# polixir/emei

Measured on AMD Instinct MI355X. Metric: env-steps/s, higher is better.
Workload: dtype f64

## Files before the change

### emei_amd/csrc/abi.hip

```cpp
#include <hip/hip_runtime.h>

#include <cmath>
#include <cstdarg>
#include <cstdio>
#include <cstring>
#include <ctime>
#include <new>

#include "launch.h"
#include "body_kernels.h"
#include "cheetah_model.h"
#include "hopper_model.h"
#include "dpend_model.h"

using namespace emei;

struct emei_env {
    emei_config cfg;
    int obs_dim, act_dim, state_dim;
    size_t real_size;
    void* state;
    int32_t* steps;
    uint32_t* episode;
    unsigned long long* done_mask;
    void* frozen_state;
    int32_t* frozen_steps;
    uint32_t* frozen_episode;
    uint64_t frozen_seed;
    unsigned long long* cap_hits;
    uint32_t* work;
    int resident_waves;
    bool has_state, frozen;
    int last_kernel;
    uint32_t* host_flag = nullptr;
    uint32_t flag_seq = 0;
    PendParams pend;
    const void* trig;
    ObsPeers peers;
};

static thread_local char g_err[512] = "";

static int fail(int code, const char* fmt, ...) {
    va_list ap;
    va_start(ap, fmt);
    vsnprintf(g_err, sizeof(g_err), fmt, ap);
// ... 60 lines not shown
    if (!out || capacity < 0) return fail(EMEI_ERR_INVALID, "emei_model_invweights: bad argument");
    double buf[32];
    int n;
    switch (env_id) {
        case EMEI_IP_REBOUND_BALANCING:
        case EMEI_IP_BOUNDARY_BALANCING:
        case EMEI_IP_REBOUND_SWINGUP:
        case EMEI_IP_BOUNDARY_SWINGUP: {
            constexpr IpModel m = ip_make_model(false);
            buf[0] = m.invw, buf[1] = m.invw_hinge, n = 2;
            break;
        }
        case EMEI_IDP_REBOUND_BALANCING:
        case EMEI_IDP_BOUNDARY_BALANCING:
        case EMEI_IDP_REBOUND_SWINGUP:
        case EMEI_IDP_BOUNDARY_SWINGUP: buf[0] = dpend::make_model(false, 0.002).invw, n = 1; break;
        case EMEI_HALFCHEETAH_RUNNING: n = cheetah::xml_invweights(buf); break;
        case EMEI_HOPPER_RUNNING: n = hopper::xml_invweights(buf); break;
        case EMEI_CARTPOLE_SWINGUP:
        case EMEI_CARTPOLE_BALANCING: return fail(EMEI_ERR_UNSUPPORTED, "emei_model_invweights: CartPole has no constraint rows");
        default: return fail(EMEI_ERR_INVALID, "unknown env_id %d", env_id);
    }
    if (n > capacity) return fail(EMEI_ERR_INVALID, "emei_model_invweights: %d values, capacity %d", n, capacity);
    memcpy(out, buf, n * sizeof(double));
    return n;
}

#include <cstddef>
#include <mutex>
namespace emei {
const void* emei_trig_table(int device) {
// ... 41 lines not shown
    p.dt = dt;
    p.dt32 = (float)dt;
    for (int i = 0; i < 4; ++i) p.init_sigma[i] = init_sigma ? init_sigma[i] : 0.f;
    p.noise_shared = noise_shared;
    const bool swingup = env_id == EMEI_IP_REBOUND_SWINGUP || env_id == EMEI_IP_BOUNDARY_SWINGUP;
    const IpModel x = ip_make_model(swingup);
    p.M11 = x.M11, p.M22 = x.M22, p.mpr = x.mpr, p.mgr = x.mp * x.gravity * x.r;
    p.gear = x.gear, p.ctrl_lo = x.ctrl_lo, p.ctrl_hi = x.ctrl_hi, p.x_lo = x.x_lo, p.x_hi = x.x_hi;
    p.phi_off = x.phi_off, p.sin_off = x.sin_off, p.cos_off = x.cos_off;
    p.invw = x.invw;
    p.tc = x.solref_tc < 2 * dt ? 2 * dt : x.solref_tc;
    p.dampratio = 1.0, p.dmin = x.dmin, p.dmax = x.dmax, p.width = x.width;
    p.limK = 1.0 / (p.dmax * p.dmax * p.tc * p.tc * p.dampratio * p.dampratio), p.limB = 2.0 / (p.dmax * p.tc);
    return p;
}

extern "C" EMEI_API int emei_create(const emei_config* cfg, emei_env** out) {
    if (!cfg || !out) return fail(EMEI_ERR_INVALID, "emei_create: null argument");
    const uint32_t size_v2a = (uint32_t)offsetof(emei_config, env_param_mask);
    const uint32_t size_v5 = (uint32_t)offsetof(emei_config, ode_method);
    if (cfg->struct_size != sizeof(emei_config) && cfg->struct_size != size_v5 && cfg->struct_size != size_v2a &&
        cfg->struct_size != EMEI_CONFIG_SIZE_V1)
        return fail(EMEI_ERR_INVALID, "emei_create: emei_config size %u, library expects %zu (or the older sizes %u / %u / %u)",
                    cfg->struct_size, sizeof(emei_config), size_v5, size_v2a, EMEI_CONFIG_SIZE_V1);
    emei_config c2;
    memset(&c2, 0, sizeof(c2));
    memcpy(&c2, cfg, cfg->struct_size);
    if (cfg->struct_size == EMEI_CONFIG_SIZE_V1)
        for (int i = 0; i < EMEI_MAX_STATE_DIM; ++i) c2.init_sigma[i] = (float)c2.init_noise;
    c2.struct_size = sizeof(emei_config);
// ... 29 lines not shown
    if (cfg->max_episode_steps < 0) return fail(EMEI_ERR_INVALID, "emei_create: max_episode_steps < 0");
    int prev_device = 0;
    HIP_TRY(hipGetDevice(&prev_device));
    HIP_TRY(hipSetDevice(cfg->device));
    struct RestoreDevice {
        int d;
        ~RestoreDevice() { (void)hipSetDevice(d); }
    } restore{prev_device};

    emei_env* h = new (std::nothrow) emei_env();
    if (!h) return fail(EMEI_ERR_INVALID, "emei_create: out of host memory");
    memset(h, 0, sizeof(*h));
    h->cfg = *cfg;
    h->obs_dim = od, h->act_dim = ad, h->state_dim = sd;
    h->real_size = cfg->precision == EMEI_PRECISION_F32 ? sizeof(float) : sizeof(double);
    const size_t n = (size_t)cfg->n_envs, n_words = (n + kWave - 1) / kWave;
    const size_t state_bytes = n * sd * h->real_size;
    hipError_t e = hipSuccess;
    if (e == hipSuccess) e = hipMalloc(&h->state, state_bytes);
    if (e == hipSuccess) e = hipMalloc((void**)&h->steps, n * sizeof(int32_t));
    if (e == hipSuccess) e = hipMalloc((void**)&h->episode, n * sizeof(uint32_t));
    if (e == hipSuccess) e = hipMalloc((void**)&h->done_mask, n_words * sizeof(unsigned long long));
    if (e == hipSuccess) e = hipMalloc(&h->frozen_state, state_bytes);
    if (e == hipSuccess) e = hipMalloc((void**)&h->frozen_steps, n * sizeof(int32_t));
    if (e == hipSuccess) e = hipMalloc((void**)&h->frozen_episode, n * sizeof(uint32_t));
    if (e == hipSuccess) e = hipMalloc((void**)&h->cap_hits, sizeof(unsigned long long));
    if (e == hipSuccess) e = hipMemset(h->cap_hits, 0, sizeof(unsigned long long));
    if (e == hipSuccess && steps_as_body(*cfg)) {
        e = hipMalloc((void**)&h->work, (2 + 2 * n_words) * sizeof(uint32_t));
        if (e == hipSuccess) e = hipMemset(h->work, 0, (2 + 2 * n_words) * sizeof(uint32_t));
// ... 1 lines not shown
    if (e == hipSuccess) e = hipMemset(h->done_mask, 0, n_words * sizeof(unsigned long long));
    if (e == hipSuccess) e = hipMemset(h->steps, 0, n * sizeof(int32_t));
    if (e == hipSuccess) e = hipMemset(h->episode, 0, n * sizeof(uint32_t));
    if (e != hipSuccess) {
        emei_destroy(h);
        return fail(EMEI_ERR_HIP, "emei_create: allocation failed: %s", hipGetErrorString(e));
    }
    if (is_pend(cfg->env_id))
        h->pend = pend_params(cfg->env_id, cfg->real_time_scale, cfg->init_sigma, cfg->noise_layout);
    h->trig = emei_trig_table(cfg->device);
    if (!h->trig) {
        emei_destroy(h);
        return fail(EMEI_ERR_HIP, "emei_create: could not build the trig table on device %d", cfg->device);
    }
    if (steps_as_body(*cfg)) {
        BodyLaunch L;
        L.op = BODY_OP_OCCUPANCY, L.env_id = cfg->env_id, L.precision = cfg->precision, L.integrator = cfg->integrator;
        L.solver = (int)cfg->solver, L.selected = &h->resident_waves;
        if (body_launch(L) != EMEI_OK) h->resident_waves = 0;
    }
    *out = h;
    return EMEI_OK;
}

extern "C" EMEI_API int emei_destroy(emei_env* h) {
    if (!h) return EMEI_OK;
    (void)hipFree(h->state);
    (void)hipFree(h->steps);
    (void)hipFree(h->episode);
    (void)hipFree(h->done_mask);
    (void)hipFree(h->frozen_state);
    (void)hipFree(h->frozen_steps);
    (void)hipFree(h->frozen_episode);
// ... 49 lines not shown
    L.freq_rate = h->cfg.freq_rate;
    L.max_episode_steps = h->cfg.max_episode_steps;
    L.seed = h->cfg.seed;
    L.env_offset = h->cfg.env_index_offset;
    L.dt = h->cfg.real_time_scale;
    L.integrator = h->cfg.integrator;
    L.solver = (int)h->cfg.solver;
    memcpy(L.noise.init, h->cfg.init_sigma, sizeof(L.noise.init));
    memcpy(L.noise.obs, h->cfg.obs_sigma, sizeof(L.noise.obs));
    L.noise.shared = h->cfg.noise_layout == EMEI_NOISE_SHARED;
    L.env_params.mask = h->cfg.env_param_mask;
    memcpy(L.env_params.v, h->cfg.env_params, sizeof(L.env_params.v));
    L.trig = h->trig;
    L.cap_hits = h->cap_hits;
    L.work = h->work, L.chunk_steps = h->cfg.rollout_chunk_steps, L.resident_waves = h->resident_waves;
    L.stream = (hipStream_t)stream;
    return L;
}

extern "C" EMEI_API int emei_reset(emei_env* h, uint64_t seed, void* stream) {
    if (!h) return fail(EMEI_ERR_INVALID, "emei_reset: null handle");
    EMEI_ON_DEVICE(h, "emei_reset");
    h->cfg.seed = seed;
    int rc;
    if (is_pend(h->cfg.env_id)) {
        PendLaunch L = pend_base(h, stream);
        L.op = PEND_OP_RESET;
        rc = pend_launch(L);
    } else {
        BodyLaunch L = body_base(h, stream);
// ... 764 lines not shown
```

### emei_amd/csrc/body_kernels.h

```cpp
#pragma once
#include "emei_device.h"

namespace emei {

struct EnvParams {
    uint32_t mask = 0;
    double v[EMEI_MAX_ENV_PARAMS] = {0};
    double get(int k, double dflt) const { return (mask >> k) & 1u ? v[k] : dflt; }
};

struct NoiseSpec {
    float init[EMEI_MAX_STATE_DIM] = {0}, obs[EMEI_MAX_STATE_DIM] = {0};
    int32_t shared = 0;
};
template <int NS>
struct NoiseArgs {
    float init[NS], obs[NS];
    int32_t shared, obs_on;
    NoiseArgs() = default;
    explicit NoiseArgs(const NoiseSpec& h) : shared(h.shared), obs_on(0) {
        for (int i = 0; i < NS; ++i) init[i] = h.init[i], obs[i] = h.obs[i], obs_on |= h.obs[i] != 0.f;
    }
};
constexpr uint64_t kObsNoiseKey = 0x6F62736E6F697365ull;
// ... 19 lines not shown
        boxmuller(r.v[2], r.v[3], z[4 * b + 2], z[4 * b + 3]);
    }
#pragma unroll
    for (int i = 0; i < NS; ++i) {
        const R d = (R)__fmul_rn(sig[i], z[i]);
        s[i] = ASSIGN ? d : s[i] + d;
    }
}
template <class Body>
__device__ __forceinline__ void body_init(typename Body::real (&s)[Body::NS], uint64_t seed, uint64_t env, uint32_t episode,
                                          const NoiseArgs<Body::NS>& ns) {
    gauss_state<typename Body::real, Body::NS, true>(s, seed, env, episode, 0u, ns.init, ns.shared != 0);
    Body::init_base(s);
}

template <class Body, bool RK4>
__device__ __forceinline__ void body_substep(typename Body::real (&s)[Body::NS], const typename Body::real (&ctrl)[Body::NA],
                                             const typename Body::Model& m, bool semi, const TrigCtx& trig,
                                             typename Body::Warm& warm) {
    using R = typename Body::real;
    constexpr int NV = Body::NS / 2;
    const R dt = (R)m.dt;
    R q[NV], v[NV], acc[NV];
#pragma unroll
    for (int i = 0; i < NV; ++i) q[i] = s[i], v[i] = s[NV + i];
    if constexpr (!RK4) {
        typename Body::Warm cold{};
        Body::accel(q, v, ctrl, m, dt, acc, trig, cold);
#pragma unroll
        for (int i = 0; i < NV; ++i) {
            const R vn = fma_r(dt, acc[i], v[i]);
            s[i] = fma_r(dt, semi ? vn : v[i], q[i]);
            s[NV + i] = vn;
        }
    } else {
        R qs[NV], vs[NV], dq[NV], dv[NV];
#pragma unroll
        for (int i = 0; i < NV; ++i) qs[i] = q[i], vs[i] = v[i], dq[i] = R(0), dv[i] = R(0);
        Body::begin_stages(warm);
        auto stage = [&](int st) __attribute__((always_inline)) {
            Body::accel(qs, vs, ctrl, m, R(0), acc, trig, warm);
            const R b = (st == 0 || st == 3) ? R(1.0 / 6.0) : R(1.0 / 3.0);
            const R h = dt * (st == 2 ? R(1) : R(0.5));
#pragma unroll
            for (int i = 0; i < NV; ++i) {
                dq[i] = fma_r(b, vs[i], dq[i]), dv[i] = fma_r(b, acc[i], dv[i]);
                qs[i] = fma_r(h, vs[i], q[i]);
// ... 34 lines not shown
    uint8_t* done_out = nullptr;
    int64_t n = 0;
    int32_t n_steps = 1, freq_rate = 1, max_episode_steps = 0;
    uint32_t flags = 0;
    uint64_t seed = 0, env_offset = 0;
    double dt = 0.002;
    int32_t integrator = 0;
    int32_t solver = 0;
    NoiseSpec noise;
    EnvParams env_params;
    const void* trig = nullptr;
    unsigned long long* cap_hits = nullptr;
    uint32_t* work = nullptr;
    int32_t chunk_steps = 0;
    int32_t resident_waves = 0;
    hipStream_t stream = nullptr;
    int* selected = nullptr;
    const double* start_rows = nullptr;
    int32_t n_candidates = 1;
    double discount = 1.0;
    double* return_out = nullptr;
    int32_t* length_out = nullptr;
    CandidateSpec cand = {};
    void* partials = nullptr;
    const float* sigma_map = nullptr;
};
int body_launch(const BodyLaunch& L);

template <class Body>
struct BodyArgs {
// ... 48 lines not shown
    }
};

template <class Body>
__host__ __device__ constexpr int rollout_block() {
#ifdef EMEI_BODY_BLOCK
    return EMEI_BODY_BLOCK;
#else
    return Body::kMinWavesPerEU == 1 ? kWave : kBlock;
#endif
}

#ifndef EMEI_WORKQUEUE
#define EMEI_WORKQUEUE 1
#endif
template <class Body, bool RK4, bool QUEUE = false>
__global__ void __launch_bounds__(rollout_block<Body>()) __attribute__((amdgpu_waves_per_eu(Body::kMinWavesPerEU)))
    body_rollout_kernel(const BodyArgs<Body> a) {
    static_assert(!QUEUE || rollout_block<Body>() == kWave, "work items are one-wave blocks");
    using R = typename Body::real;
    constexpr int NS = Body::NS, NO = Body::NO, NA = Body::NA;
    constexpr int kBlock = rollout_block<Body>();
    constexpr int kWaves = kBlock / kWave;
    constexpr int kActVec = (kWave * NA + 3) / 4, kObsVec = (kWave * NO + 3) / 4;
    constexpr int kActIt = (kActVec + kWave - 1) / kWave, kObsIt = (kObsVec + kWave - 1) / kWave;
    __shared__ __attribute__((aligned(16))) float act_s[kWaves][kActIt * kWave * 4];
    __shared__ __attribute__((aligned(16))) float obs_s[kWaves][kObsIt * kWave * 4];
    __shared__ SinCosEntry trig_s[kTrigTableSize];
    stage_trig_table<kBlock>(trig_s, a.trig);
    TrigCtx trig;
    trig.tab = trig_s;
    __shared__ R scratch_s[(Body::kScratchPerLane > 0 ? Body::kScratchPerLane : 1) * (Body::kScratchPerLane > 0 ? kBlock : 1)];
    if constexpr (Body::kScratchPerLane > 0) trig.scratch = scratch_s;
    trig.scratch_stride = kBlock;
// ... 48 lines not shown
    const int wave_envs = (int)min((int64_t)kWave, n - i0);
    const bool active = i < n;

    R s[NS];
    int32_t steps = 0;
    uint32_t episode = 0;
    if (active) {
#pragma unroll
        for (int k = 0; k < NS; ++k) s[k] = a.state[(int64_t)k * n + i];
        steps = a.steps[i];
        episode = a.episode[i];
    } else {
        Body::park(s);
    }
    const bool auto_reset = (a.flags & EMEI_FLAG_AUTO_RESET) != 0;
    const bool obs_noise = a.noise.obs_on != 0;
    uint32_t done = 0;
    R spare[Body::kSpareReset ? NS : 1];
    bool have_spare = false;

    float4 av[kActIt];
    auto fetch_actions = [&](int t) __attribute__((always_inline)) {
        const float* base = a.actions + ((int64_t)t * n + i0) * NA;
        const bool fast = wave_envs == kWave && (((uintptr_t)base) & 15u) == 0;
#pragma unroll
        for (int c = 0; c < kActIt; ++c) {
            const int vec = c * kWave + lane;
            av[c] = make_float4(0.f, 0.f, 0.f, 0.f);
            if (fast) {
                if (vec < kActVec) av[c] = ((const float4*)base)[vec];
            } else {
// ... 17 lines not shown
        } else {
#pragma unroll
            for (int c = 0; c < kActIt; ++c) ((float4*)act_s[wv])[c * kWave + lane] = av[c];
            wave_lds_fence();
#pragma unroll
            for (int k = 0; k < NA; ++k) ctrl[k] = (R)act_s[wv][lane * NA + k];
            wave_lds_fence();
            if (t + 1 < t_end) fetch_actions(t + 1);
        }

        R pre[NS];
#pragma unroll
        for (int k = 0; k < NS; ++k) pre[k] = s[k];
        typename Body::Warm warm{};
        for (int k = 0; k < a.freq_rate; ++k) {
            body_substep<Body, RK4>(s, ctrl, a.m, a.semi != 0, trig, warm);
            if (obs_noise)
                gauss_state<R, NS, false>(s, a.seed ^ kObsNoiseKey, a.env_offset + (uint64_t)i, episode,
                                          ((uint32_t)steps * (uint32_t)a.freq_rate + (uint32_t)k) * (uint32_t)((NS + 3) / 4),
                                          a.noise.obs, a.noise.shared != 0);
        }
        EMEI_MARK(step_io);
        float o[NO];
        R rew;
        bool term;
        Body::outputs(s, pre, ctrl, a.m, a.freq_rate, o, rew, term, trig);
        ++steps;
        const bool trunc = (a.max_episode_steps > 0) & (steps >= a.max_episode_steps);
        done = active ? ((term ? EMEI_DONE_TERMINAL : 0u) | (trunc ? EMEI_DONE_TRUNCATED : 0u)) : 0u;

        if (a.obs_out) {
            float* mine = &obs_s[wv][lane * NO];
#pragma unroll
            for (int k = 0; k < NO; ++k) mine[k] = o[k];
            wave_lds_fence();
// ... 249 lines not shown
                if constexpr (!DRAWN) {
                    ret_out[j] = ret;
                    len_out[j] = t + 1;
                    if (final_obs) {
#pragma unroll
                        for (int k = 0; k < NO; ++k) final_obs[j * NO + k] = o[k];
                    }
                }
            }
        }
        if (__ballot(live) == 0ull) break;
    }
    if constexpr (DRAWN) plan_reduce_wave(j, nk, i, n_cand, ret, len, partials);
    if constexpr (DRAWN && KEEP) {
        if (active) ret_out[j] = ret;
    }
}

template <class Body>
static int launch_body(const BodyLaunch& L) {
    using R = typename Body::real;
    const typename Body::Model m = Body::make_model(L.dt, L.env_params);
    dim3 grid((unsigned)((L.n + kBlock - 1) / kBlock));
    dim3 rgrid((unsigned)((L.n + rollout_block<Body>() - 1) / rollout_block<Body>()));
    switch (L.op) {
        case BODY_OP_ROLLOUT: {
            BodyArgs<Body> a;
            a.state = (R*)L.state, a.steps = L.steps, a.episode = L.episode, a.done_mask = L.done_mask;
            a.actions = (const float*)L.actions, a.obs_out = L.obs_out, a.reward_out = L.reward_out, a.done_out = L.done_out;
            a.n = L.n, a.n_steps = L.n_steps, a.freq_rate = L.freq_rate, a.max_episode_steps = L.max_episode_steps;
// ... 3 lines not shown
            a.cap_hits = L.cap_hits;
            a.work = nullptr, a.chunk_steps = 0, a.n_waves = rgrid.x, a.n_items = 0;
            if constexpr (rollout_block<Body>() == kWave && EMEI_WORKQUEUE != 0) {
                int cs = L.chunk_steps;
                if (cs == 0) cs = (L.resident_waves > 0 && (int64_t)rgrid.x > L.resident_waves) ? -((kGuidedMin << 4) | kGuidedShift) : 0;
                else if (cs <= -100) cs = -(((-cs / 100) << 4) | max(1, min(-cs % 100, 6)));
                else if (cs < 0) cs = 0;
                const unsigned n_chunks = cs != 0 ? WorkQueue::count_chunks(L.n_steps, cs) : 1u;
                if (L.work && n_chunks > 1 && (uint64_t)rgrid.x * n_chunks < (1ull << 31)) {
                    static_assert(WorkQueue::kProgress == WorkQueue::kTicket + 1, "one memset");
                    if (hipMemsetAsync(L.work + WorkQueue::kTicket, 0, (size_t)(1 + rgrid.x) * sizeof(uint32_t), L.stream) != hipSuccess)
                        return EMEI_ERR_HIP;
                    a.work = L.work, a.chunk_steps = cs, a.n_items = rgrid.x * n_chunks;
                    const unsigned workers = L.resident_waves > 0 ? (unsigned)L.resident_waves : 1024u;
                    rgrid.x = min(workers, a.n_items);
                    if (L.integrator == EMEI_INTEG_RK4)
                        hipLaunchKernelGGL((body_rollout_kernel<Body, true, true>), rgrid, dim3(kWave), 0, L.stream, a);
                    else
                        hipLaunchKernelGGL((body_rollout_kernel<Body, false, true>), rgrid, dim3(kWave), 0, L.stream, a);
                }
            }
            if (!a.work) {
                if (L.integrator == EMEI_INTEG_RK4)
                    hipLaunchKernelGGL((body_rollout_kernel<Body, true>), rgrid, dim3(rollout_block<Body>()), 0, L.stream, a);
                else
                    hipLaunchKernelGGL((body_rollout_kernel<Body, false>), rgrid, dim3(rollout_block<Body>()), 0, L.stream, a);
            }
            if (L.selected)
                *L.selected = a.work ? (L.integrator == EMEI_INTEG_RK4 ? EMEI_KERNEL_BODY_RK4_CHUNKED : EMEI_KERNEL_BODY_CHUNKED)
                                     : (L.integrator == EMEI_INTEG_RK4 ? EMEI_KERNEL_BODY_RK4 : EMEI_KERNEL_BODY);
            break;
        }
        case BODY_OP_OCCUPANCY: {
            int dev = 0, cus = 0, nb = 0;
            if (hipGetDevice(&dev) != hipSuccess || hipDeviceGetAttribute(&cus, hipDeviceAttributeMultiprocessorCount, dev) != hipSuccess)
                return EMEI_ERR_HIP;
            hipError_t e;
            if constexpr (rollout_block<Body>() == kWave && EMEI_WORKQUEUE != 0) {
                e = L.integrator == EMEI_INTEG_RK4
                        ? hipOccupancyMaxActiveBlocksPerMultiprocessor(&nb, body_rollout_kernel<Body, true, true>, rollout_block<Body>(), 0)
                        : hipOccupancyMaxActiveBlocksPerMultiprocessor(&nb, body_rollout_kernel<Body, false, true>, rollout_block<Body>(), 0);
            } else {
                e = L.integrator == EMEI_INTEG_RK4
                        ? hipOccupancyMaxActiveBlocksPerMultiprocessor(&nb, body_rollout_kernel<Body, true>, rollout_block<Body>(), 0)
                        : hipOccupancyMaxActiveBlocksPerMultiprocessor(&nb, body_rollout_kernel<Body, false>, rollout_block<Body>(), 0);
            }
            if (e != hipSuccess) return EMEI_ERR_HIP;
            if (L.selected) *L.selected = nb * cus * (rollout_block<Body>() / kWave);
            return EMEI_OK;
        }
        case BODY_OP_RESET:
            hipLaunchKernelGGL(body_reset_kernel<Body>, grid, dim3(kBlock), 0, L.stream, (R*)L.state, L.steps, L.episode,
                               L.n, L.seed, L.env_offset, NoiseArgs<Body::NS>(L.noise));
            break;
        case BODY_OP_GET_OBS:
            hipLaunchKernelGGL(body_get_obs_kernel<Body>, grid, dim3(kBlock), 0, L.stream, (const R*)L.state, L.obs_f64,
                               L.n, m);
            break;
        case BODY_OP_INIT_OBS:
            hipLaunchKernelGGL(body_init_obs_kernel<Body>, grid, dim3(kBlock), 0, L.stream, L.env_index, L.episode_in,
                               L.obs_out, L.n, L.seed, L.env_offset, NoiseArgs<Body::NS>(L.noise), m);
// ... 110 lines not shown
```

### emei_amd/csrc/cheetah_model.h

```cpp
#pragma once
#include <cmath>
#include <cstring>
#include <type_traits>

#include "constexpr_math.h"
#include "emei_device.h"

namespace emei {
namespace cheetah {

constexpr int NV = 9;
enum { P_BFOOT = 0, P_BSHIN = 1, P_BTHIGH = 2, P_FFOOT = 3, P_FSHIN = 4, P_FTHIGH = 5, P_TORSO = 6, P_X = 7, P_Z = 8 };

__host__ __device__ constexpr bool nz(int i, int j) { return i >= 6 || (i / 3) == (j / 3); }

struct Model {
    double sx[7], sz[7], diag[7];
    double d_tb[2], d_tf[2], d_bt_bs[2], d_bs_bf[2], d_ft_fs[2], d_fs_ff[2];
    double mtot, gravity, z0;
    double stiff[6], damp[6], arm[6], lo[6], hi[6], gear[6];
    double geom_end[16][2];
    double radius, friction;
    double cK, cB, c_dmin, c_dmax, c_width;
    double lK, lB, l_dmin, l_dmax, l_width;
// ... 1124 lines not shown
    qacc[6] = a[P_FTHIGH] - a[P_TORSO], qacc[7] = a[P_FSHIN] - a[P_FTHIGH], qacc[8] = a[P_FFOOT] - a[P_FSHIN];
}

}

template <typename R, int SOLVER = EMEI_SOLVER_NEWTON>
struct CheetahBody {
    using real = R;
    using Model = cheetah::Model;
    static constexpr int kMinWavesPerEU = 1;
#ifndef EMEI_CHEETAH_UNROLL_RK4
#define EMEI_CHEETAH_UNROLL_RK4 1
#endif
    static constexpr bool kUnrollRK4 = EMEI_CHEETAH_UNROLL_RK4 != 0;
    static constexpr int kScratchPerLane = SOLVER == EMEI_SOLVER_NEWTON ? cheetah::kDualSlots * cheetah::kSlotFields : 0;
    static constexpr bool kHasCtrlCost = true;
    static constexpr bool kObsIsState = true;
    static constexpr bool kSpareReset = false;
    static constexpr bool kStreamOutputs = false;
    static constexpr int NS = 18, NO = 18, NA = 6;
    static Model make_model(double dt, const EnvParams& ep) {
        Model m = cheetah::cheetah_make_model(dt);
        m.w_forward = ep.get(EMEI_PARAM_FORWARD_REWARD_WEIGHT, 1.0), m.w_ctrl = ep.get(EMEI_PARAM_CTRL_COST_WEIGHT, 0.1);
        return m;
    }

    struct WarmNone {};
    using Warm = std::conditional_t<SOLVER == EMEI_SOLVER_SWEEP1, WarmNone, cheetah::NewtonWarm<R>>;
    __device__ __forceinline__ static void begin_stages(Warm&) {}
    __device__ __forceinline__ static void accel(const R (&q)[cheetah::NV], const R (&v)[cheetah::NV], const R (&ctrl)[NA],
// ... 51 lines not shown
```

### emei_amd/csrc/dpend_model.h

```cpp
#pragma once
#include <cmath>
#include <cstring>

#include "emei_device.h"

namespace emei {
namespace dpend {

struct Model {
    double s1z, s2z, diag1, diag2, L1, mtot;
    double gx, gz, gear, x_lo, x_hi, margin, invw;
    double K, B, dmin, dmax, width;
    double dt, phi_off;
};

namespace host {
inline double capsule_mass(double rho, double r, double half) { return rho * (M_PI * r * r * 2 * half + 4.0 / 3.0 * M_PI * r * r * r); }
inline double capsule_inertia_perp(double rho, double r, double half) {
    double h = 2 * half, mcyl = rho * M_PI * r * r * h, msph = rho * 4.0 / 3.0 * M_PI * r * r * r;
    return mcyl * (3 * r * r + h * h) / 12 + msph * (2 * r * r / 5 + h * h / 4 + 3 * h * r / 8);
}
}

struct Xml {
    double rho, cart_r, cart_half, pole_r, pole_half, L1, gx, gz, gear, ctrl_lo, ctrl_hi, x_lo, x_hi, margin, solref_tc, dmin, dmax, width;
};
constexpr Xml kXml = {1000.0, 0.1, 0.1,
                      0.045, 0.3, 0.6,
                      1e-5, 9.81,
                      500.0, -1.0, 1.0,
                      -3.0, 3.0, 0.01,
                      0.02, 0.9, 0.95, 0.001};

inline Model make_model(bool swingup, double dt) {
    Model m;
    memset(&m, 0, sizeof(m));
    const double rho = kXml.rho;
    const double mc = host::capsule_mass(rho, kXml.cart_r, kXml.cart_half);
    const double mp = host::capsule_mass(rho, kXml.pole_r, kXml.pole_half);
    const double Ip = host::capsule_inertia_perp(rho, kXml.pole_r, kXml.pole_half);
    const double lc = kXml.pole_half, L1 = kXml.L1;
    m.s1z = mp * lc + mp * L1, m.s2z = mp * lc;
    m.diag1 = Ip + mp * lc * lc + mp * L1 * L1, m.diag2 = Ip + mp * lc * lc;
    m.L1 = L1, m.mtot = mc + 2 * mp;
    m.gx = kXml.gx, m.gz = kXml.gz;
    m.gear = kXml.gear;
    m.x_lo = kXml.x_lo, m.x_hi = kXml.x_hi, m.margin = kXml.margin;
    const double a = m.mtot, b = m.s1z, c = m.s2z, d = m.diag1, e = L1 * m.s2z, f = m.diag2;
    const double det = a * (d * f - e * e) - b * (b * f - e * c) + c * (b * e - d * c);
    m.invw = (d * f - e * e) / det;
    const double tc = kXml.solref_tc < 2 * dt ? 2 * dt : kXml.solref_tc, dmax = kXml.dmax;
    m.K = 1.0 / (dmax * dmax * tc * tc), m.B = 2.0 / (dmax * tc);
    m.dmin = kXml.dmin, m.dmax = dmax, m.width = kXml.width;
    m.dt = dt;
    m.phi_off = swingup ? M_PI : 0.0;
    return m;
}

inline int xml_constants(double* out) {
    const double mc = host::capsule_mass(kXml.rho, kXml.cart_r, kXml.cart_half), mp = host::capsule_mass(kXml.rho, kXml.pole_r, kXml.pole_half);
    const double v[17] = {kXml.gx, kXml.gz, mc, mp, host::capsule_inertia_perp(kXml.rho, kXml.pole_r, kXml.pole_half), kXml.pole_half,
                          kXml.L1, kXml.gear, kXml.ctrl_lo, kXml.ctrl_hi, kXml.x_lo, kXml.x_hi, kXml.margin, kXml.solref_tc, kXml.dmin,
                          kXml.dmax, kXml.width};
    for (int i = 0; i < 17; ++i) out[i] = v[i];
    return 17;
}

}

template <int VARIANT, typename R>
struct DPendBody {
    using real = R;
    using Model = dpend::Model;
    static constexpr int kMinWavesPerEU = 1;
    static constexpr bool kUnrollRK4 = false;
    static constexpr int kScratchPerLane = 0;
    static constexpr bool kHasCtrlCost = false;
    static constexpr bool kObsIsState = false;
    static constexpr bool kSpareReset = true;
    static constexpr bool kStreamOutputs = true;
    static constexpr int NS = 6, NO = 6, NA = 1;
    static Model make_model(double dt, const EnvParams&) { return dpend::make_model(VARIANT >= 2, dt); }

    struct Warm {};
    __device__ __forceinline__ static void begin_stages(Warm&) {}
    __device__ __forceinline__ static void accel(const R (&q)[3], const R (&v)[3], const R (&ctrl)[NA], const Model& m, R,
                                                 R (&qacc)[3], const TrigCtx& trig, Warm&) {
        const R phi1 = q[1] + (R)m.phi_off, phi2 = phi1 + q[2];
        const R w1 = v[1], w2 = v[1] + v[2];
        R s1, c1, s2, c2;
        sincos_ctx(trig, phi1, s1, c1);
        sincos_ctx(trig, phi2, s2, c2);
        const R S1x = (R)m.s1z * s1, S1z = (R)m.s1z * c1, S2x = (R)m.s2z * s2, S2z = (R)m.s2z * c2;
        const R Dx = (R)m.L1 * s1, Dz = (R)m.L1 * c1;
        const R M12 = fma_r(Dx, S2x, Dz * S2z);
        const R u = ctrl[0] < R(dpend::kXml.ctrl_lo) ? R(dpend::kXml.ctrl_lo) : (ctrl[0] > R(dpend::kXml.ctrl_hi) ? R(dpend::kXml.ctrl_hi) : ctrl[0]);
        const R w1s = w1 * w1, w2s = w2 * w2;
        R fx = (R)m.gear * u + (R)m.mtot * (R)m.gx + w1s * S1x + w2s * S2x;
        R f1 = (R)m.gx * S1z + (R)m.gz * S1x + w2s * fma_r(S2x, Dz, -(S2z * Dx));
        R f2 = (R)m.gx * S2z + (R)m.gz * S2x + w1s * fma_r(Dx, S2z, -(Dz * S2x));
        const R a = (R)m.mtot, b = S1z, c = S2z, d = (R)m.diag1, e = M12, f = (R)m.diag2;
        const R if_ = rcp1_r(f);
        const R le = e * if_, lc = c * if_;
        const R d1 = fma_r(-le, e, d), b1 = fma_r(-le, c, b), a1 = fma_r(-lc, c, a);
        const R id1 = rcp1_r(d1);
        const R lb = b1 * id1;
        const R a2 = fma_r(-lb, b1, a1);
        const R ia2 = rcp1_r(a2);
        R ax, a1_, a2_;
        {
            const R y1 = fma_r(-le, f2, f1);
            const R yx = fma_r(-lb, y1, fma_r(-lc, f2, fx));
            ax = yx * ia2;
            a1_ = fma_r(-lb, ax, y1 * id1);
            a2_ = fma_r(-le, a1_, fma_r(-lc, ax, f2 * if_));
        }
        static_assert(dpend::kXml.x_lo == -dpend::kXml.x_hi, "symmetric slider range");
        const R ax_abs = abs_r(q[0]);
        if (ax_abs > (R)(m.x_hi - m.margin)) {
            const R nJ = copysign_r(R(1), q[0]);
            const R n1 = fma_r((R)m.B, v[0], ax);
            const R wx = ia2, w1_ = -lb * ia2, w2_ = fma_r(lb, le, -lc) * ia2;
            auto finish = [&](R Kimp, R Kimp_edge, R Rr) __attribute__((always_inline)) {
                const R num = fma_r(nJ, n1, fma_r(Kimp, ax_abs, -Kimp_edge));
                const R g = nJ * fmax_r(num * rcp1_r(wx + Rr), R(0));
                ax = fma_r(-wx, g, ax);
                a1_ = fma_r(-w1_, g, a1_);
                a2_ = fma_r(-w2_, g, a2_);
            };
            const R edge = (R)(m.x_hi - m.margin);
            const R Kfull = (R)m.K * (R)m.dmax;
            const bool full = !(ax_abs < (R)(m.x_hi - m.margin + m.width));
            if (__builtin_expect(__ballot(!full) != 0ull, 0)) {
                const R xx = (ax_abs - edge) * (R)(1.0 / m.width), u1 = R(1) - xx;
                const R y = xx <= R(0.5) ? R(2) * xx * xx : fma_r(R(-2) * u1, u1, R(1));
                const R imp = fma_r(y, (R)(m.dmax - m.dmin), (R)m.dmin);
                const R Kimp = full ? Kfull : (R)m.K * imp;
                finish(Kimp, Kimp * edge, full ? (R)((1.0 - m.dmax) / m.dmax) * (R)m.invw : (R(1) - imp) * (R)m.invw * rcp1_r(imp));
            } else {
                finish(Kfull, Kfull * edge, (R)((1.0 - m.dmax) / m.dmax) * (R)m.invw);
            }
        }
        qacc[0] = ax, qacc[1] = a1_, qacc[2] = a2_ - a1_;
    }

    template <typename T>
    __device__ __forceinline__ static T quirk_wrap(T th) {
        const T pi = T(3.141592653589793);
        return pymod_pos(th + pi, T(2), T(0.5)) * pi - pi;
    }
    template <typename T, typename SC>
    __device__ __forceinline__ static void reward_terminal(const T (&o)[NO], const Model& m, T& rew, bool& term, SC sc) {
        T sa, ca, sb, cb;
        sc(o[1], sa, ca);
        sc(o[1] + o[2], sb, cb);
        const T y = ca + cb;
        bool fin = true;
#pragma unroll
        for (int k = 0; k < NO; ++k) fin &= finite_r(o[k]);
        const bool inx = ((T)m.x_lo < o[0]) & (o[0] < (T)m.x_hi);
        if (VARIANT == 0) rew = T(1), term = !((y >= T(1.5)) & fin);
        else if (VARIANT == 1) rew = T(1), term = !((y >= T(0)) & inx & fin);
        else if (VARIANT == 2) rew = (T(2) - y) / T(4), term = !fin;
        else rew = (T(2) - y) / T(4) - (T(5e-3) * o[4] * o[4] + T(1e-4) * o[5] * o[5]), term = !(inx & fin);
    }
    __device__ __forceinline__ static void outputs(const R (&s)[NS], const R (&pre)[NS], const R (&ctrl)[NA], const Model& m,
                                                   int freq_rate, float (&o)[NO], R& rew, bool& term, const TrigCtx& trig) {
        R ob[NO] = {s[0], quirk_wrap(s[1]), quirk_wrap(s[2]), s[3], s[4], s[5]};
        reward_terminal(ob, m, rew, term, [&](R x, R& sn, R& cs) { sincos_ctx(trig, x, sn, cs); });
#pragma unroll
        for (int k = 0; k < NO; ++k) o[k] = (float)ob[k];
    }
    __device__ __forceinline__ static void init_base(R (&)[NS]) {}
    __device__ __forceinline__ static void park(R (&s)[NS]) {
#pragma unroll
// ... 28 lines not shown
```

### emei_amd/csrc/hopper_model.h

```cpp
#pragma once
#include <cmath>
#include <cstring>
#include <type_traits>

#include "cheetah_model.h"
#include "emei_device.h"

namespace emei {
namespace hopper {

constexpr int NV = 6, NL = 4;
enum { L_FOOT = 0, L_LEG = 1, L_THIGH = 2, L_TORSO = 3, P_X = 4, P_Z = 5 };
constexpr int kGeomLink[4] = {L_TORSO, L_THIGH, L_LEG, L_FOOT};

struct Model {
    double sx[NL], sz[NL], diag[NL];
    double d[NL][2];
    double mtot, gravity, z0;
    double damp[3], arm[3], lo[3], hi[3], gear[3];
    double geom_end[8][2];
    double radius[4], friction[4], margin;
    double cK, cB, c_dmin, c_dmax, c_width;
    double lK, lB, l_dmin, l_dmax, l_width;
    double dt;
// ... 805 lines not shown
    }
    EMEI_MARK(nw_out);
    qacc[0] = a[P_X], qacc[1] = a[P_Z], qacc[2] = a[L_TORSO];
    qacc[3] = hs(a[L_THIGH] - a[L_TORSO]), qacc[4] = hs(a[L_LEG] - a[L_THIGH]), qacc[5] = hs(a[L_FOOT] - a[L_LEG]);
}

}

template <typename R, int SOLVER = EMEI_SOLVER_NEWTON>
struct HopperBody {
    using real = R;
    using Model = hopper::Model;
    static constexpr int kMinWavesPerEU = SOLVER == EMEI_SOLVER_SWEEP1 ? 2 : 1;
    static constexpr bool kUnrollRK4 = false;
    static constexpr int kScratchPerLane = 0;
    static constexpr bool kHasCtrlCost = true;
    static constexpr bool kObsIsState = true;
    static constexpr bool kSpareReset = false;
    static constexpr bool kStreamOutputs = false;
    static constexpr int NS = 12, NO = 12, NA = 3;
    static Model make_model(double dt, const EnvParams& ep) {
        Model m = hopper::make_model(dt);
        m.w_forward = ep.get(EMEI_PARAM_FORWARD_REWARD_WEIGHT, 1.0), m.w_ctrl = ep.get(EMEI_PARAM_CTRL_COST_WEIGHT, 1e-3);
        m.healthy_reward = ep.get(EMEI_PARAM_HEALTHY_REWARD, 1.0);
        m.terminate_when_unhealthy = ep.get(EMEI_PARAM_TERMINATE_WHEN_UNHEALTHY, 1.0) != 0.0;
        m.st_lo = ep.get(EMEI_PARAM_HEALTHY_STATE_LO, -100.0), m.st_hi = ep.get(EMEI_PARAM_HEALTHY_STATE_HI, 100.0);
        m.z_lo = ep.get(EMEI_PARAM_HEALTHY_Z_LO, 0.7), m.z_hi = ep.get(EMEI_PARAM_HEALTHY_Z_HI, (double)INFINITY);
        return m;
    }

// ... 75 lines not shown
```

### emei_amd/csrc/ipend_model.h

```cpp
#pragma once
#include <cmath>
#include <cstring>

#include "emei_device.h"
#include "pendulum_envs.h"

namespace emei {
namespace ipend {

struct Model {
    double M11, M22, mpr, mgr, gear, ctrl_lo, ctrl_hi, x_lo, x_hi;
    double phi_off, sin_off, cos_off;
    double invw, K, B, dmin, dmax, width;
    double dt;
};

namespace host {
inline double capsule_mass(double rho, double r, double half) { return rho * (M_PI * r * r * 2 * half + 4.0 / 3.0 * M_PI * r * r * r); }
inline double capsule_inertia_perp(double rho, double r, double half) {
    double h = 2 * half, mcyl = rho * M_PI * r * r * h, msph = rho * 4.0 / 3.0 * M_PI * r * r * r;
    return mcyl * (3 * r * r + h * h) / 12 + msph * (2 * r * r / 5 + h * h / 4 + 3 * h * r / 8);
}
}

// ... 12 lines not shown
    m.K = 1.0 / (dmax * dmax * tc * tc), m.B = 2.0 / (dmax * tc);
    m.dmin = x.dmin, m.dmax = dmax, m.width = x.width;
    m.dt = dt;
    return m;
}

}

template <int VARIANT, typename R>
struct InvPendBody {
    using real = R;
    using Model = ipend::Model;
    static constexpr int kMinWavesPerEU = 1;
    static constexpr bool kUnrollRK4 = true;
    static constexpr int kScratchPerLane = 0;
    static constexpr bool kHasCtrlCost = false;
    static constexpr bool kObsIsState = true;
    static constexpr bool kSpareReset = true;
    static constexpr bool kStreamOutputs = true;
    static constexpr int NS = 4, NO = 4, NA = 1;
    static Model make_model(double dt, const EnvParams&) { return ipend::make_model(VARIANT >= 2, dt); }

    struct Warm {};
    __device__ __forceinline__ static void begin_stages(Warm&) {}
    __device__ __forceinline__ static void accel(const R (&q)[2], const R (&v)[2], const R (&ctrl)[NA], const Model& m, R,
                                                 R (&qacc)[2], const TrigCtx& trig, Warm&) {
        R sn, cs;
        sincos_ctx(trig, q[1] + (R)m.phi_off, sn, cs);
        const R M11 = (R)m.M11, M22 = (R)m.M22, M12 = (R)m.mpr * cs;
        const R u = ctrl[0] < (R)m.ctrl_lo ? (R)m.ctrl_lo : (ctrl[0] > (R)m.ctrl_hi ? (R)m.ctrl_hi : ctrl[0]);
// ... 78 lines not shown
```

Before: 280.3 billion.

## Add lean Euler rollout kernel for double pendulum with compile-time constants

Adds a specialised rollout kernel variant, on by default unless EMEI_BODY_LEAN=0, for the double pendulum under Euler integration with no observation noise. It fixes the semi-implicit flag at compile time and drops the per-substep noise branch. The dpend model is split so the mass and geometry constants become constexpr values instead of runtime struct fields, which shrinks the kernel argument and lets the compiler fold them. This costs an extra kernel instantiation, and the variant is only valid when noise is zero.

```diff
diff --git a/emei_amd/csrc/abi.hip b/emei_amd/csrc/abi.hip
--- a/emei_amd/csrc/abi.hip
+++ b/emei_amd/csrc/abi.hip
@@ -3,6 +3,7 @@
 #include <cmath>
 #include <cstdarg>
 #include <cstdio>
+#include <cstdlib>
 #include <cstring>
 #include <ctime>
 #include <new>
@@ -30,6 +31,7 @@
     unsigned long long* cap_hits;
     uint32_t* work;
     int resident_waves;
+    int body_lean;
     bool has_state, frozen;
     int last_kernel;
     uint32_t* host_flag = nullptr;
@@ -120,7 +122,11 @@
         case EMEI_IDP_REBOUND_BALANCING:
         case EMEI_IDP_BOUNDARY_BALANCING:
         case EMEI_IDP_REBOUND_SWINGUP:
-        case EMEI_IDP_BOUNDARY_SWINGUP: buf[0] = dpend::make_model(false, 0.002).invw, n = 1; break;
+        case EMEI_IDP_BOUNDARY_SWINGUP: {
+            constexpr dpend::Const c = dpend::make_const();
+            buf[0] = c.invw, n = 1;
+            break;
+        }
         case EMEI_HALFCHEETAH_RUNNING: n = cheetah::xml_invweights(buf); break;
         case EMEI_HOPPER_RUNNING: n = hopper::xml_invweights(buf); break;
         case EMEI_CARTPOLE_SWINGUP:
@@ -192,6 +198,8 @@
     p.limK = 1.0 / (p.dmax * p.dmax * p.tc * p.tc * p.dampratio * p.dampratio), p.limB = 2.0 / (p.dmax * p.tc);
     return p;
 }
+
+static BodyLaunch body_base(emei_env* h, void* stream);
 
 extern "C" EMEI_API int emei_create(const emei_config* cfg, emei_env** out) {
     if (!cfg || !out) return fail(EMEI_ERR_INVALID, "emei_create: null argument");
@@ -251,6 +259,8 @@
     h->cfg = *cfg;
     h->obs_dim = od, h->act_dim = ad, h->state_dim = sd;
     h->real_size = cfg->precision == EMEI_PRECISION_F32 ? sizeof(float) : sizeof(double);
+    const char* lean_env = getenv("EMEI_BODY_LEAN");
+    h->body_lean = !(lean_env && strcmp(lean_env, "0") == 0);
     const size_t n = (size_t)cfg->n_envs, n_words = (n + kWave - 1) / kWave;
     const size_t state_bytes = n * sd * h->real_size;
     hipError_t e = hipSuccess;
@@ -282,9 +292,8 @@
         return fail(EMEI_ERR_HIP, "emei_create: could not build the trig table on device %d", cfg->device);
     }
     if (steps_as_body(*cfg)) {
-        BodyLaunch L;
-        L.op = BODY_OP_OCCUPANCY, L.env_id = cfg->env_id, L.precision = cfg->precision, L.integrator = cfg->integrator;
-        L.solver = (int)cfg->solver, L.selected = &h->resident_waves;
+        BodyLaunch L = body_base(h, nullptr);
+        L.op = BODY_OP_OCCUPANCY, L.selected = &h->resident_waves;
         if (body_launch(L) != EMEI_OK) h->resident_waves = 0;
     }
     *out = h;
@@ -364,6 +373,7 @@
     L.trig = h->trig;
     L.cap_hits = h->cap_hits;
     L.work = h->work, L.chunk_steps = h->cfg.rollout_chunk_steps, L.resident_waves = h->resident_waves;
+    L.lean = h->body_lean;
     L.stream = (hipStream_t)stream;
     return L;
 }
diff --git a/emei_amd/csrc/body_kernels.h b/emei_amd/csrc/body_kernels.h
--- a/emei_amd/csrc/body_kernels.h
+++ b/emei_amd/csrc/body_kernels.h
@@ -57,13 +57,14 @@
     Body::init_base(s);
 }
 
-template <class Body, bool RK4>
+template <class Body, bool RK4, int SEMI = -1>
 __device__ __forceinline__ void body_substep(typename Body::real (&s)[Body::NS], const typename Body::real (&ctrl)[Body::NA],
                                              const typename Body::Model& m, bool semi, const TrigCtx& trig,
                                              typename Body::Warm& warm) {
     using R = typename Body::real;
     constexpr int NV = Body::NS / 2;
     const R dt = (R)m.dt;
+    const bool use_vn = SEMI < 0 ? semi : SEMI != 0;
     R q[NV], v[NV], acc[NV];
 #pragma unroll
     for (int i = 0; i < NV; ++i) q[i] = s[i], v[i] = s[NV + i];
@@ -73,7 +74,7 @@
 #pragma unroll
         for (int i = 0; i < NV; ++i) {
             const R vn = fma_r(dt, acc[i], v[i]);
-            s[i] = fma_r(dt, semi ? vn : v[i], q[i]);
+            s[i] = fma_r(dt, use_vn ? vn : v[i], q[i]);
             s[NV + i] = vn;
         }
     } else {
@@ -138,6 +139,7 @@
     uint32_t* work = nullptr;
     int32_t chunk_steps = 0;
     int32_t resident_waves = 0;
+    int32_t lean = 1;
     hipStream_t stream = nullptr;
     int* selected = nullptr;
     const double* start_rows = nullptr;
@@ -216,10 +218,11 @@
 #ifndef EMEI_WORKQUEUE
 #define EMEI_WORKQUEUE 1
 #endif
-template <class Body, bool RK4, bool QUEUE = false>
+template <class Body, bool RK4, bool QUEUE = false, bool LEAN = false>
 __global__ void __launch_bounds__(rollout_block<Body>()) __attribute__((amdgpu_waves_per_eu(Body::kMinWavesPerEU)))
     body_rollout_kernel(const BodyArgs<Body> a) {
     static_assert(!QUEUE || rollout_block<Body>() == kWave, "work items are one-wave blocks");
+    static_assert(!LEAN || !RK4, "the lean form is the Euler position override");
     using R = typename Body::real;
     constexpr int NS = Body::NS, NO = Body::NO, NA = Body::NA;
     constexpr int kBlock = rollout_block<Body>();
@@ -298,7 +301,7 @@
         Body::park(s);
     }
     const bool auto_reset = (a.flags & EMEI_FLAG_AUTO_RESET) != 0;
-    const bool obs_noise = a.noise.obs_on != 0;
+    [[maybe_unused]] const bool obs_noise = !LEAN && a.noise.obs_on != 0;
     uint32_t done = 0;
     R spare[Body::kSpareReset ? NS : 1];
     bool have_spare = false;
@@ -346,11 +349,15 @@
         for (int k = 0; k < NS; ++k) pre[k] = s[k];
         typename Body::Warm warm{};
         for (int k = 0; k < a.freq_rate; ++k) {
-            body_substep<Body, RK4>(s, ctrl, a.m, a.semi != 0, trig, warm);
-            if (obs_noise)
-                gauss_state<R, NS, false>(s, a.seed ^ kObsNoiseKey, a.env_offset + (uint64_t)i, episode,
-                                          ((uint32_t)steps * (uint32_t)a.freq_rate + (uint32_t)k) * (uint32_t)((NS + 3) / 4),
-                                          a.noise.obs, a.noise.shared != 0);
+            if constexpr (LEAN) {
+                body_substep<Body, false, 0>(s, ctrl, a.m, false, trig, warm);
+            } else {
+                body_substep<Body, RK4>(s, ctrl, a.m, a.semi != 0, trig, warm);
+                if (obs_noise)
+                    gauss_state<R, NS, false>(s, a.seed ^ kObsNoiseKey, a.env_offset + (uint64_t)i, episode,
+                                              ((uint32_t)steps * (uint32_t)a.freq_rate + (uint32_t)k) * (uint32_t)((NS + 3) / 4),
+                                              a.noise.obs, a.noise.shared != 0);
+            }
         }
         EMEI_MARK(step_io);
         float o[NO];
@@ -630,6 +637,18 @@
     if constexpr (DRAWN) plan_reduce_wave(j, nk, i, n_cand, ret, len, partials);
     if constexpr (DRAWN && KEEP) {
         if (active) ret_out[j] = ret;
+    }
+}
+
+template <class Body>
+static bool lean_launch(const BodyLaunch& L) {
+    if constexpr (!Body::kLeanRollout) {
+        return false;
+    } else {
+        if (!L.lean || L.integrator != EMEI_INTEG_EULER) return false;
+        for (int i = 0; i < Body::NS; ++i)
+            if (L.noise.obs[i] != 0.f) return false;
+        return true;
     }
 }
 
@@ -663,17 +682,23 @@
                     a.work = L.work, a.chunk_steps = cs, a.n_items = rgrid.x * n_chunks;
                     const unsigned workers = L.resident_waves > 0 ? (unsigned)L.resident_waves : 1024u;
                     rgrid.x = min(workers, a.n_items);
-                    if (L.integrator == EMEI_INTEG_RK4)
+                    if (L.integrator == EMEI_INTEG_RK4) {
                         hipLaunchKernelGGL((body_rollout_kernel<Body, true, true>), rgrid, dim3(kWave), 0, L.stream, a);
-                    else
+                    } else if (lean_launch<Body>(L)) {
+                        hipLaunchKernelGGL((body_rollout_kernel<Body, false, true, Body::kLeanRollout>), rgrid, dim3(kWave), 0, L.stream, a);
+                    } else {
                         hipLaunchKernelGGL((body_rollout_kernel<Body, false, true>), rgrid, dim3(kWave), 0, L.stream, a);
+                    }
                 }
             }
             if (!a.work) {
-                if (L.integrator == EMEI_INTEG_RK4)
+                if (L.integrator == EMEI_INTEG_RK4) {
                     hipLaunchKernelGGL((body_rollout_kernel<Body, true>), rgrid, dim3(rollout_block<Body>()), 0, L.stream, a);
-                else
+                } else if (lean_launch<Body>(L)) {
+                    hipLaunchKernelGGL((body_rollout_kernel<Body, false, false, Body::kLeanRollout>), rgrid, dim3(rollout_block<Body>()), 0, L.stream, a);
+                } else {
                     hipLaunchKernelGGL((body_rollout_kernel<Body, false>), rgrid, dim3(rollout_block<Body>()), 0, L.stream, a);
+                }
             }
             if (L.selected)
                 *L.selected = a.work ? (L.integrator == EMEI_INTEG_RK4 ? EMEI_KERNEL_BODY_RK4_CHUNKED : EMEI_KERNEL_BODY_CHUNKED)
@@ -684,16 +709,11 @@
             int dev = 0, cus = 0, nb = 0;
             if (hipGetDevice(&dev) != hipSuccess || hipDeviceGetAttribute(&cus, hipDeviceAttributeMultiprocessorCount, dev) != hipSuccess)
                 return EMEI_ERR_HIP;
-            hipError_t e;
-            if constexpr (rollout_block<Body>() == kWave && EMEI_WORKQUEUE != 0) {
-                e = L.integrator == EMEI_INTEG_RK4
-                        ? hipOccupancyMaxActiveBlocksPerMultiprocessor(&nb, body_rollout_kernel<Body, true, true>, rollout_block<Body>(), 0)
-                        : hipOccupancyMaxActiveBlocksPerMultiprocessor(&nb, body_rollout_kernel<Body, false, true>, rollout_block<Body>(), 0);
-            } else {
-                e = L.integrator == EMEI_INTEG_RK4
-                        ? hipOccupancyMaxActiveBlocksPerMultiprocessor(&nb, body_rollout_kernel<Body, true>, rollout_block<Body>(), 0)
-                        : hipOccupancyMaxActiveBlocksPerMultiprocessor(&nb, body_rollout_kernel<Body, false>, rollout_block<Body>(), 0);
-            }
+            constexpr bool kQ = rollout_block<Body>() == kWave && EMEI_WORKQUEUE != 0;
+            auto occupancy = [&](auto kernel) { return hipOccupancyMaxActiveBlocksPerMultiprocessor(&nb, kernel, rollout_block<Body>(), 0); };
+            const hipError_t e = L.integrator == EMEI_INTEG_RK4 ? occupancy(body_rollout_kernel<Body, true, kQ>)
+                                 : lean_launch<Body>(L)         ? occupancy(body_rollout_kernel<Body, false, kQ, Body::kLeanRollout>)
+                                                                : occupancy(body_rollout_kernel<Body, false, kQ>);
             if (e != hipSuccess) return EMEI_ERR_HIP;
             if (L.selected) *L.selected = nb * cus * (rollout_block<Body>() / kWave);
             return EMEI_OK;
diff --git a/emei_amd/csrc/cheetah_model.h b/emei_amd/csrc/cheetah_model.h
--- a/emei_amd/csrc/cheetah_model.h
+++ b/emei_amd/csrc/cheetah_model.h
@@ -1162,6 +1162,7 @@
 #endif
     static constexpr bool kUnrollRK4 = EMEI_CHEETAH_UNROLL_RK4 != 0;
     static constexpr int kScratchPerLane = SOLVER == EMEI_SOLVER_NEWTON ? cheetah::kDualSlots * cheetah::kSlotFields : 0;
+    static constexpr bool kLeanRollout = false;
     static constexpr bool kHasCtrlCost = true;
     static constexpr bool kObsIsState = true;
     static constexpr bool kSpareReset = false;
diff --git a/emei_amd/csrc/dpend_model.h b/emei_amd/csrc/dpend_model.h
--- a/emei_amd/csrc/dpend_model.h
+++ b/emei_amd/csrc/dpend_model.h
@@ -1,22 +1,24 @@
 #pragma once
 #include <cmath>
-#include <cstring>
 
 #include "emei_device.h"
 
 namespace emei {
 namespace dpend {
 
-struct Model {
+struct Const {
+    double mc, mp, Ip;
     double s1z, s2z, diag1, diag2, L1, mtot;
     double gx, gz, gear, x_lo, x_hi, margin, invw;
-    double K, B, dmin, dmax, width;
-    double dt, phi_off;
+    double dmin, dmax, width;
+};
+struct Model {
+    double K, B, dt;
 };
 
 namespace host {
-inline double capsule_mass(double rho, double r, double half) { return rho * (M_PI * r * r * 2 * half + 4.0 / 3.0 * M_PI * r * r * r); }
-inline double capsule_inertia_perp(double rho, double r, double half) {
+constexpr double capsule_mass(double rho, double r, double half) { return rho * (M_PI * r * r * 2 * half + 4.0 / 3.0 * M_PI * r * r * r); }
+constexpr double capsule_inertia_perp(double rho, double r, double half) {
     double h = 2 * half, mcyl = rho * M_PI * r * r * h, msph = rho * 4.0 / 3.0 * M_PI * r * r * r;
     return mcyl * (3 * r * r + h * h) / 12 + msph * (2 * r * r / 5 + h * h / 4 + 3 * h * r / 8);
 }
@@ -32,14 +34,14 @@
                       -3.0, 3.0, 0.01,
                       0.02, 0.9, 0.95, 0.001};
 
-inline Model make_model(bool swingup, double dt) {
-    Model m;
-    memset(&m, 0, sizeof(m));
+constexpr Const make_const() {
+    Const m{};
     const double rho = kXml.rho;
     const double mc = host::capsule_mass(rho, kXml.cart_r, kXml.cart_half);
     const double mp = host::capsule_mass(rho, kXml.pole_r, kXml.pole_half);
     const double Ip = host::capsule_inertia_perp(rho, kXml.pole_r, kXml.pole_half);
     const double lc = kXml.pole_half, L1 = kXml.L1;
+    m.mc = mc, m.mp = mp, m.Ip = Ip;
     m.s1z = mp * lc + mp * L1, m.s2z = mp * lc;
     m.diag1 = Ip + mp * lc * lc + mp * L1 * L1, m.diag2 = Ip + mp * lc * lc;
     m.L1 = L1, m.mtot = mc + 2 * mp;
@@ -49,17 +51,21 @@
     const double a = m.mtot, b = m.s1z, c = m.s2z, d = m.diag1, e = L1 * m.s2z, f = m.diag2;
     const double det = a * (d * f - e * e) - b * (b * f - e * c) + c * (b * e - d * c);
     m.invw = (d * f - e * e) / det;
+    m.dmin = kXml.dmin, m.dmax = kXml.dmax, m.width = kXml.width;
+    return m;
+}
+
+inline Model make_model(double dt) {
+    Model m;
     const double tc = kXml.solref_tc < 2 * dt ? 2 * dt : kXml.solref_tc, dmax = kXml.dmax;
     m.K = 1.0 / (dmax * dmax * tc * tc), m.B = 2.0 / (dmax * tc);
-    m.dmin = kXml.dmin, m.dmax = dmax, m.width = kXml.width;
     m.dt = dt;
-    m.phi_off = swingup ? M_PI : 0.0;
     return m;
 }
 
 inline int xml_constants(double* out) {
-    const double mc = host::capsule_mass(kXml.rho, kXml.cart_r, kXml.cart_half), mp = host::capsule_mass(kXml.rho, kXml.pole_r, kXml.pole_half);
-    const double v[17] = {kXml.gx, kXml.gz, mc, mp, host::capsule_inertia_perp(kXml.rho, kXml.pole_r, kXml.pole_half), kXml.pole_half,
+    constexpr Const c = make_const();
+    const double v[17] = {kXml.gx, kXml.gz, c.mc, c.mp, c.Ip, kXml.pole_half,
                           kXml.L1, kXml.gear, kXml.ctrl_lo, kXml.ctrl_hi, kXml.x_lo, kXml.x_hi, kXml.margin, kXml.solref_tc, kXml.dmin,
                           kXml.dmax, kXml.width};
     for (int i = 0; i < 17; ++i) out[i] = v[i];
@@ -79,28 +85,33 @@
     static constexpr bool kObsIsState = false;
     static constexpr bool kSpareReset = true;
     static constexpr bool kStreamOutputs = true;
+    static constexpr bool kLeanRollout = true;
     static constexpr int NS = 6, NO = 6, NA = 1;
-    static Model make_model(double dt, const EnvParams&) { return dpend::make_model(VARIANT >= 2, dt); }
+    static constexpr double kPhiOff = VARIANT >= 2 ? M_PI : 0.0;
+    static Model make_model(double dt, const EnvParams&) { return dpend::make_model(dt); }
 
     struct Warm {};
     __device__ __forceinline__ static void begin_stages(Warm&) {}
     __device__ __forceinline__ static void accel(const R (&q)[3], const R (&v)[3], const R (&ctrl)[NA], const Model& m, R,
                                                  R (&qacc)[3], const TrigCtx& trig, Warm&) {
-        const R phi1 = q[1] + (R)m.phi_off, phi2 = phi1 + q[2];
+        const R phi1 = q[1] + (R)kPhiOff, phi2 = phi1 + q[2];
         const R w1 = v[1], w2 = v[1] + v[2];
+        constexpr dpend::Const kc = dpend::make_const();
         R s1, c1, s2, c2;
         sincos_ctx(trig, phi1, s1, c1);
         sincos_ctx(trig, phi2, s2, c2);
-        const R S1x = (R)m.s1z * s1, S1z = (R)m.s1z * c1, S2x = (R)m.s2z * s2, S2z = (R)m.s2z * c2;
-        const R Dx = (R)m.L1 * s1, Dz = (R)m.L1 * c1;
+        const R S1x = (R)kc.s1z * s1, S1z = (R)kc.s1z * c1, S2x = (R)kc.s2z * s2, S2z = (R)kc.s2z * c2;
+        const R Dx = (R)kc.L1 * s1, Dz = (R)kc.L1 * c1;
         const R M12 = fma_r(Dx, S2x, Dz * S2z);
         const R u = ctrl[0] < R(dpend::kXml.ctrl_lo) ? R(dpend::kXml.ctrl_lo) : (ctrl[0] > R(dpend::kXml.ctrl_hi) ? R(dpend::kXml.ctrl_hi) : ctrl[0]);
         const R w1s = w1 * w1, w2s = w2 * w2;
-        R fx = (R)m.gear * u + (R)m.mtot * (R)m.gx + w1s * S1x + w2s * S2x;
-        R f1 = (R)m.gx * S1z + (R)m.gz * S1x + w2s * fma_r(S2x, Dz, -(S2z * Dx));
-        R f2 = (R)m.gx * S2z + (R)m.gz * S2x + w1s * fma_r(Dx, S2z, -(Dz * S2x));
-        const R a = (R)m.mtot, b = S1z, c = S2z, d = (R)m.diag1, e = M12, f = (R)m.diag2;
-        const R if_ = rcp1_r(f);
+        R fx = (R)kc.gear * u + (R)kc.mtot * (R)kc.gx + w1s * S1x + w2s * S2x;
+        R f1 = (R)kc.gx * S1z + (R)kc.gz * S1x + w2s * fma_r(S2x, Dz, -(S2z * Dx));
+        R f2 = (R)kc.gx * S2z + (R)kc.gz * S2x + w1s * fma_r(Dx, S2z, -(Dz * S2x));
+        const R a = (R)kc.mtot, b = S1z, c = S2z, d = (R)kc.diag1, e = M12, f = (R)kc.diag2;
+        R f_rt = f;
+        asm("" : "+s"(f_rt));
+        const R if_ = rcp1_r(f_rt);
         const R le = e * if_, lc = c * if_;
         const R d1 = fma_r(-le, e, d), b1 = fma_r(-le, c, b), a1 = fma_r(-lc, c, a);
         const R id1 = rcp1_r(d1);
@@ -117,7 +128,7 @@
         }
         static_assert(dpend::kXml.x_lo == -dpend::kXml.x_hi, "symmetric slider range");
         const R ax_abs = abs_r(q[0]);
-        if (ax_abs > (R)(m.x_hi - m.margin)) {
+        if (ax_abs > (R)(kc.x_hi - kc.margin)) {
             const R nJ = copysign_r(R(1), q[0]);
             const R n1 = fma_r((R)m.B, v[0], ax);
             const R wx = ia2, w1_ = -lb * ia2, w2_ = fma_r(lb, le, -lc) * ia2;
@@ -128,17 +139,17 @@
                 a1_ = fma_r(-w1_, g, a1_);
                 a2_ = fma_r(-w2_, g, a2_);
             };
-            const R edge = (R)(m.x_hi - m.margin);
-            const R Kfull = (R)m.K * (R)m.dmax;
-            const bool full = !(ax_abs < (R)(m.x_hi - m.margin + m.width));
+            const R edge = (R)(kc.x_hi - kc.margin);
+            const R Kfull = (R)m.K * (R)kc.dmax;
+            const bool full = !(ax_abs < (R)(kc.x_hi - kc.margin + kc.width));
             if (__builtin_expect(__ballot(!full) != 0ull, 0)) {
-                const R xx = (ax_abs - edge) * (R)(1.0 / m.width), u1 = R(1) - xx;
+                const R xx = (ax_abs - edge) * (R)(1.0 / kc.width), u1 = R(1) - xx;
                 const R y = xx <= R(0.5) ? R(2) * xx * xx : fma_r(R(-2) * u1, u1, R(1));
-                const R imp = fma_r(y, (R)(m.dmax - m.dmin), (R)m.dmin);
+                const R imp = fma_r(y, (R)(kc.dmax - kc.dmin), (R)kc.dmin);
                 const R Kimp = full ? Kfull : (R)m.K * imp;
-                finish(Kimp, Kimp * edge, full ? (R)((1.0 - m.dmax) / m.dmax) * (R)m.invw : (R(1) - imp) * (R)m.invw * rcp1_r(imp));
+                finish(Kimp, Kimp * edge, full ? (R)((1.0 - kc.dmax) / kc.dmax) * (R)kc.invw : (R(1) - imp) * (R)kc.invw * rcp1_r(imp));
             } else {
-                finish(Kfull, Kfull * edge, (R)((1.0 - m.dmax) / m.dmax) * (R)m.invw);
+                finish(Kfull, Kfull * edge, (R)((1.0 - kc.dmax) / kc.dmax) * (R)kc.invw);
             }
         }
         qacc[0] = ax, qacc[1] = a1_, qacc[2] = a2_ - a1_;
@@ -158,7 +169,7 @@
         bool fin = true;
 #pragma unroll
         for (int k = 0; k < NO; ++k) fin &= finite_r(o[k]);
-        const bool inx = ((T)m.x_lo < o[0]) & (o[0] < (T)m.x_hi);
+        const bool inx = ((T)dpend::kXml.x_lo < o[0]) & (o[0] < (T)dpend::kXml.x_hi);
         if (VARIANT == 0) rew = T(1), term = !((y >= T(1.5)) & fin);
         else if (VARIANT == 1) rew = T(1), term = !((y >= T(0)) & inx & fin);
         else if (VARIANT == 2) rew = (T(2) - y) / T(4), term = !fin;
diff --git a/emei_amd/csrc/hopper_model.h b/emei_amd/csrc/hopper_model.h
--- a/emei_amd/csrc/hopper_model.h
+++ b/emei_amd/csrc/hopper_model.h
@@ -843,6 +843,7 @@
     static constexpr int kMinWavesPerEU = SOLVER == EMEI_SOLVER_SWEEP1 ? 2 : 1;
     static constexpr bool kUnrollRK4 = false;
     static constexpr int kScratchPerLane = 0;
+    static constexpr bool kLeanRollout = false;
     static constexpr bool kHasCtrlCost = true;
     static constexpr bool kObsIsState = true;
     static constexpr bool kSpareReset = false;
diff --git a/emei_amd/csrc/ipend_model.h b/emei_amd/csrc/ipend_model.h
--- a/emei_amd/csrc/ipend_model.h
+++ b/emei_amd/csrc/ipend_model.h
@@ -50,6 +50,7 @@
     static constexpr int kMinWavesPerEU = 1;
     static constexpr bool kUnrollRK4 = true;
     static constexpr int kScratchPerLane = 0;
+    static constexpr bool kLeanRollout = false;
     static constexpr bool kHasCtrlCost = false;
     static constexpr bool kObsIsState = true;
     static constexpr bool kSpareReset = true;
```

Result: no change. 280.4 billion, median of 2 (+0.1%).
